# NingZhang1/pyscf_isdf

Measured on AMD Instinct MI355X. Metric: isdf_build_plus_get_jk_wall_time, lower is better.
Workload: dtype f64

## Files before the change

### include/mi355_isdf.h

```cpp
#ifndef MI355_ISDF_H
#define MI355_ISDF_H

#include <stdint.h>

#ifdef __cplusplus
extern "C" {
#endif

typedef struct isdf_ctx* isdf_handle;

#define ISDF_OK 0
#define ISDF_ERR_ARG 1
#define ISDF_ERR_HIP 2
#define ISDF_ERR_LIB 3
#define ISDF_ERR_NUM 4

int isdf_abi_version(void);

int isdf_create(int device_id, isdf_handle* out);
int isdf_destroy(isdf_handle h);
int isdf_set_stream(isdf_handle h, void* hip_stream);
const char* isdf_last_error(isdf_handle h);
int64_t isdf_workspace_bytes(isdf_handle h);
int isdf_release_workspace(isdf_handle h);
// ... 244 lines not shown
int isdf_dot(isdf_handle h, const double* d_x, const double* d_y, int64_t n, double* result);

int isdf_pack_table_pm(isdf_handle h, const double* d_tab, const int32_t mesh[3], const int32_t* d_idx, int npts, double scale,
                       double* d_s, double* d_a, int64_t ldx);
int isdf_herm_kscale_nt(isdf_handle h, int M, int N, int64_t K, double alpha, const double* d_A, int64_t lda, const double* d_B,
                        int64_t ldb, const double* d_s, const double* d_a, double beta, double* d_Cre, double* d_Cim, int64_t ldc);

int isdf_thc_pair(isdf_handle h, int P, const double* d_Xo, int64_t ldo, int no, const double* d_so, const double* d_Xv, int64_t ldv,
                  int nv, const double* d_sv, double* d_A, int64_t lda);
int isdf_trace_sq(isdf_handle h, int n, const double* d_B, int64_t ldb, double* result);

int isdf_gemm_nt(isdf_handle h, int M, int N, int64_t K, double alpha, const double* d_A, int64_t lda,
                 const double* d_B, int64_t ldb, const double* d_kscale, double beta, double* d_C,
                 int64_t ldc);

int isdf_gemm_nt_had3(isdf_handle h, int M, int N, int64_t K, double alpha, const double* d_A, int64_t lda, const double* d_H,
                      int64_t ldh, const double* d_B, int64_t ldb, int64_t bstride, double beta, double* d_C, int64_t ldc,
                      int64_t cstride);

int isdf_gemm_nn_had(isdf_handle h, int M, int64_t N, int K, double alpha, const double* d_A, int64_t lda, const double* d_H,
                     int64_t ldh, const double* d_B, int64_t ldb, double beta, double* d_C, int64_t ldc);

#ifdef __cplusplus
}
#endif
#endif
```

### pyscf_isdf_amd/backend.py

```python
import ctypes
import os
import numpy as np
import torch
from . import lib as _lib

_vp = ctypes.c_void_p


def _np_ptr(a):
    return a.ctypes.data_as(_vp)


class HipBackend:
    name = 'hip-gfx950'

    def __init__(self, device=0):
        if not torch.cuda.is_available():
            raise _lib.IsdfError('no GPU visible to torch; the ISDF path has no CPU fallback')
        self.device = torch.device('cuda', device)
        torch.cuda.set_device(self.device)
        self.handle = _lib.Handle(device)
        if os.environ.get('ISDF_TRSM') == 'subst':
            self.set_option('trsm_substitution', 1)
        if os.environ.get('ISDF_OWN_FFT') in ('0', '1', '2'):
# ... 464 lines not shown
                         B.stride(0), float(beta), self._p(C), C.stride(0))

    def hadamard_rows(self, X, Y):
        self._stream()
        self.handle.call('isdf_hadamard_rows', self._p(X), X.stride(0), self._p(Y), Y.stride(0), X.shape[0], X.shape[1])

    def gemm_nt(self, A, B, C, alpha=1.0, beta=0.0, kscale=None):
        self._stream()
        M, K = A.shape
        N = B.shape[0]
        assert B.shape[1] == K and tuple(C.shape) == (M, N) and A.stride(1) == 1 and B.stride(1) == 1 and C.stride(1) == 1
        ks = self._p(kscale) if kscale is not None else _vp(0)
        self.handle.call('isdf_gemm_nt', M, N, K, float(alpha), self._p(A), A.stride(0), self._p(B), B.stride(0), ks,
                         float(beta), self._p(C), C.stride(0))

    def gemm_nt_had3(self, A, H, B3, C3, alpha=1.0, beta=0.0):
        self._stream()
        M, K = A.shape
        N = B3.shape[1]
        assert tuple(B3.shape) == (3, N, K) and tuple(C3.shape) == (3, M, N) and A.stride(1) == 1 and B3.stride(2) == 1 and C3.stride(2) == 1
        assert H is None or (tuple(H.shape) == (M, K) and H.stride(1) == 1)
        self.handle.call('isdf_gemm_nt_had3', M, N, K, float(alpha), self._p(A), A.stride(0), self._p(H) if H is not None else _vp(0),
                         H.stride(0) if H is not None else 0, self._p(B3), B3.stride(1), B3.stride(0), float(beta), self._p(C3),
                         C3.stride(1), C3.stride(0))

    def gemm_nn_had(self, A, H, B, C, alpha=1.0, beta=0.0):
        self._stream()
        M, K = A.shape
        N = B.shape[1]
        assert tuple(B.shape) == (K, N) and tuple(H.shape) == (K, N) and tuple(C.shape) == (M, N)
# ... 310 lines not shown
```

### pyscf_isdf_amd/csrc/common.h

```cpp
#pragma once
#include <hip/hip_runtime.h>
#include <rocblas/rocblas.h>
#include <rocsolver/rocsolver.h>
#include <hipfft/hipfft.h>
#include <cstdint>
#include <cstdio>
#include <cstring>
#include <string>
#include <vector>
#include <map>
#include "../../include/mi355_isdf.h"

struct FftPlan {
  hipfftHandle fwd = 0, bwd = 0;
  size_t work_bytes = 0;
};

struct ProfRec {
  hipEvent_t e0 = nullptr, e1 = nullptr;
};
struct ProfEntry {
  std::vector<ProfRec> recs;
  double work = 0.0;
  double ms = 0.0;
// ... 9 lines not shown
};

struct isdf_ctx {
  int profiling = 0;
  std::map<std::string, ProfEntry> prof;
  int device = 0;
  hipStream_t stream = nullptr;
  rocblas_handle blas = nullptr;
  std::string err;
  std::map<std::vector<int>, FftPlan> plans;
  std::map<std::string, std::pair<void*, size_t>> ws;
  int num_cu = 256;
  int trsm_substitution = 0;
  int own_fft = 2;
  int gemm_nn_own = 0;
  int attr_gemm_b = 0, attr_gemm_nn = 0, attr_gemm_nn_had = 0, attr_gram_tri = 0, attr_herm = 0, attr_thc_pair = 0;
  int cand_gram = 1;
  int conv_pipe = 1;
  int conv_sub_rows = 0;
  int gram_pivot_tpb = 256;
  int gram_compact = 1;
  int gram_compact_permille = 875;
  int block_apply_waves = 16;
  int block_apply_reg = 1;
  double coul_omega = 0.0;
  double coul_rc = 0.0;
  int coul_sphere = 0;
  WsKernel wsk;
};

int isdf_fail(isdf_handle h, int code, const char* fmt, ...);
// ... 56 lines not shown
    if (hipEventCreate(&rec.e0) != hipSuccess || hipEventCreate(&rec.e1) != hipSuccess) { ent = nullptr; return; }
    (void)hipEventRecord(rec.e0, h->stream);
  }
  ~ProfScope() {
    if (!ent) return;
    (void)hipEventRecord(rec.e1, h->stream);
    ent->recs.push_back(rec);
  }
};

int gemm_nt_f64(isdf_handle h, int M, int N, int64_t K, double alpha, const double* A, int64_t lda,
                const double* B, int64_t ldb, double beta, double* C, int64_t ldc);
int gemm_nt_f64_scaled(isdf_handle h, int M, int N, int64_t K, double alpha, const double* A, int64_t lda,
                       const double* B, int64_t ldb, const double* kscale, double beta, double* C,
                       int64_t ldc);
int trsm_lower_left(isdf_handle h, bool trans, int m, int64_t n, const double* L, int64_t ldl, double* X, int64_t ldx);
int trsm_lower_right(isdf_handle h, bool trans, int m, int64_t n, const double* L, int64_t ldl, double* X, int64_t ldx);
int block_forward_solve(isdf_handle h, const double* D, int64_t ldd, int nblk, const int32_t* blk_off_host, double* X,
                        int64_t ldx, int64_t n, bool own_columns = false);
int block_apply_inverse(isdf_handle h, const double* Dinv, int64_t ldd, int nblk, const int32_t* blk_off_host, double* X,
                        int64_t ldx, int64_t n, bool square_input = false);
int transpose_rm(isdf_handle h, const double* src, int64_t lds, int64_t rows, int64_t cols, double* dst, int64_t ldd);
int tri_left(isdf_handle h, bool trans, int m, int64_t n, const double* L, int64_t ldl, double* X, int64_t ldx);
int tri_right(isdf_handle h, bool trans, int m, int64_t n, const double* L, int64_t ldl, double* X, int64_t ldx);
bool gemm_nn_f64_supported(isdf_handle h, int64_t M, int64_t N, int64_t K, const double* A, int64_t lda, const double* B,
                           int64_t ldb);
int gemm_nn_f64(isdf_handle h, int64_t M, int64_t N, int64_t K, const double* A, int64_t lda, const double* B, int64_t ldb,
                double* C, int64_t ldc, bool square);
int gemm_rm(isdf_handle h, char opA, char opB, int64_t M, int64_t N, int64_t K, double alpha,
            const double* A, int64_t lda, const double* B, int64_t ldb, double beta, double* C,
// ... 11 lines not shown
```

### pyscf_isdf_amd/csrc/gemm_f64.hip

```cpp
#include "common.h"
#include "gemm_tile.h"
#include <cstdlib>

int gemm_rm(isdf_handle h, char opA, char opB, int64_t M, int64_t N, int64_t K, double alpha,
            const double* A, int64_t lda, const double* B, int64_t ldb, double beta, double* C,
            int64_t ldc) {
  ARG_CHECK(h, M < 2147483647LL && N < 2147483647LL && K < 2147483647LL && lda < 2147483647LL &&
                   ldb < 2147483647LL && ldc < 2147483647LL);
  const rocblas_operation ta = (opA == 'N') ? rocblas_operation_none : rocblas_operation_transpose;
  const rocblas_operation tb = (opB == 'N') ? rocblas_operation_none : rocblas_operation_transpose;
  ProfScope ps(h, "rocblas_dgemm[flop]", 2.0 * M * N * (double)K);
  BLAS_TRY(h, rocblas_dgemm(h->blas, tb, ta, (rocblas_int)N, (rocblas_int)M, (rocblas_int)K, &alpha, B,
                            (rocblas_int)ldb, A, (rocblas_int)lda, &beta, C, (rocblas_int)ldc));
  return ISDF_OK;
}

namespace {

constexpr int BM = 128, BN = 128, BK = 16;
constexpr int LDT = 17;
constexpr int TPB = 256;

struct GemmArgs {
  const double* A; int64_t lda;
  const double* B; int64_t ldb;
  const double* kscale;
  double* P;
  int64_t ldp, slab_stride;
  int M, N;
  int64_t K, kslab;
  int ntm, ntn, nslab;
  int64_t nunits, nunits_pad;
  double alpha, beta;
  int direct;
};

#define ISDF_SLAB_STORE                                                                       \
  {                                                                                           \
    double* q = out + (int64_t)row * g.ldp + col;                                             \
    const double v = acc[i][j][r];                                                            \
    if (g.direct) *q = (g.beta == 0.0) ? g.alpha * v : g.alpha * v + g.beta * (*q);           \
    else *q = v;                                                                              \
  }

#define ISDF_MFMA16(AF, BF)                                                                   \
    _Pragma("unroll") for (int i = 0; i < 4; ++i)                                             \
      _Pragma("unroll") for (int j = 0; j < 4; ++j)                                           \
        acc[i][j] = __builtin_amdgcn_mfma_f64_16x16x4f64(AF[i], BF[j], acc[i][j], 0, 0, 0);
#define ISDF_ISSUE(XMASK, NX) _Pragma("unroll") for (int q_ = 0; q_ < 8; ++q_) {              \
    __builtin_amdgcn_sched_group_barrier(0x008, 2, 0); __builtin_amdgcn_sched_group_barrier(0x100, 1, 0);                \
    if (q_ < (NX)) __builtin_amdgcn_sched_group_barrier(XMASK, 1, 0); }

template <bool FAST>
__global__ __launch_bounds__(TPB, 2) void gemm_nt_mfma_kernel(GemmArgs g) {
  __shared__ double sA[2][BM * LDT];
  __shared__ double sB[2][BN * LDT];

  const int64_t unit = xcd_unit(g.nunits_pad);
  if (unit >= g.nunits) return;
  const Tile t = decode_tile(unit, g.ntm, g.ntn);
  const KRange kr = slab_range(t.slab, g.kslab, g.K);
  const int64_t k0 = kr.k0, k1 = kr.k1;
  const int nchunks = (int)((k1 - k0 + BK - 1) / BK);

  const int tid = threadIdx.x;
  const int lane = tid & 63, wave = tid >> 6;
  const int wm = wave >> 1, wn = wave & 1;

  const int srow = tid >> 3;
  const int sseg = tid & 7;
  const int arow0 = t.tm * BM + srow, brow0 = t.tn * BN + srow;
  const int mlast = g.M - 1, nlast = g.N - 1;
  const double* __restrict__ Ag = g.A;
  const double* __restrict__ Bg = g.B;
  const int64_t lda = g.lda, ldb = g.ldb;
// ... 59 lines not shown
    ISDF_FRAGS(3, a1, b1)
    ISDF_MFMA16(a0, b0)
    ISDF_MFMA16(a1, b1)
    if (c + 1 < nchunks) ISDF_STORE_CHUNK(buf ^ 1)
    __syncthreads();
  }
  double* out = g.P + (int64_t)t.slab * g.slab_stride;
  ISDF_STORE_ACC(4, 4, t.tm * BM + wm * 64, t.tn * BN + wn * 64, g.M, g.N, ISDF_SLAB_STORE)
#undef ISDF_LOAD_ONE
#undef ISDF_LOAD_CHUNK
#undef ISDF_STORE_ONE
#undef ISDF_STORE_CHUNK
#undef ISDF_FRAGS
}

constexpr int BM2 = 256;
constexpr int TPB2 = 512;

template <bool SCALED>
__device__ __forceinline__ void tile_256x128(const double* A, int64_t lda, const double* B, int64_t ldb, const double* kscale,
                                             int M, int N, int tm, int tn, int64_t k0, int nchunks, double* smem, d4 (&acc)[4][4]) {
  double* sA = smem;
  double* sB = smem + 2 * BM2 * LDT;
  const int last = nchunks - 1;

  const int tid = threadIdx.x;
  const int lane = tid & 63, wave = tid >> 6;
  const int wm = wave >> 1, wn = wave & 1;
  const int srow = tid >> 3;
  const int sseg = tid & 7;
// ... 81 lines not shown
    ISDF_CHUNKB(1, ISDF_LOADB(min(c + 3, last), ya0, ya1, ya2, ya3, yb0, yb1), ISDF_STOREB(0, xa0, xa1, xa2, xa3, xb0, xb1))
  }
#undef ISDF_LOADB
#undef ISDF_ST1
#undef ISDF_STOREB
#undef ISDF_FRAGQ
#undef ISDF_CHUNKB
}

template <bool SCALED>
__global__ __launch_bounds__(TPB2, 2) void gemm_nt_mfma_kernel_b(GemmArgs g) {
  extern __shared__ double smem[];
  const int64_t unit = xcd_unit(g.nunits_pad);
  if (unit >= g.nunits) return;
  const Tile t = decode_tile(unit, g.ntm, g.ntn);
  const KRange kr = slab_range(t.slab, g.kslab, g.K);
  d4 acc[4][4];
  tile_256x128<SCALED>(g.A, g.lda, g.B, g.ldb, g.kscale, g.M, g.N, t.tm, t.tn, kr.k0, (int)((kr.k1 - kr.k0) / BK), smem, acc);
  const int lane = threadIdx.x & 63, wave = threadIdx.x >> 6;
  double* out = g.P + (int64_t)t.slab * g.slab_stride;
  ISDF_STORE_ACC(4, 4, t.tm * BM2 + (wave >> 1) * 64, t.tn * BN + (wave & 1) * 64, g.M, g.N, ISDF_SLAB_STORE)
}

struct GramTriArgs {
  const double* X; int64_t ldx; int K;
  const GramTriUnit* units;
  const int64_t* blk_off;
  int64_t row0;
  const int64_t* tri_off;
  double* S;
// ... 6 lines not shown
  if (unit >= t.nunits) return;
  const GramTriUnit u = t.units[unit];
  const int64_t r0 = t.blk_off[u.blk];
  const double* X = t.X + (r0 - t.row0) * t.ldx;
  const int m = (int)(t.blk_off[u.blk + 1] - r0);
  const int64_t ldp = (int64_t)(u.tm + 1) * BM2;
  double* S = t.S + t.tri_off[u.blk] + (gram_tri_row((int64_t)u.tm * BM2) - (int64_t)u.tm * BM2 * ldp);
  d4 acc[4][4];
  tile_256x128<false>(X, t.ldx, X, t.ldx, nullptr, m, m, u.tm, u.tn, 0, t.K / BK, smem, acc);
  const int lane = threadIdx.x & 63, wave = threadIdx.x >> 6;
  ISDF_STORE_ACC(4, 4, u.tm * BM2 + (wave >> 1) * 64, u.tn * BN + (wave & 1) * 64, m, m, S[(int64_t)row * ldp + col] = acc[i][j][r];)
}

constexpr int TPBD = 256;

template <bool SCALED>
__global__ __launch_bounds__(TPBD, 2) void gemm_nt_mfma_kernel_d(GemmArgs g) {
  __shared__ double sB[2][BN * LDT];
  const int64_t unit = xcd_unit(g.nunits_pad);
  if (unit >= g.nunits) return;
  const Tile t = decode_tile(unit, g.ntm, g.ntn);
  const int tm = t.tm, tn = t.tn;
  const KRange kr = slab_range(t.slab, g.kslab, g.K);
  const int64_t k0 = kr.k0;
  const int nchunks = (int)((kr.k1 - k0) / BK);
  const int last = nchunks - 1;

  const int tid = threadIdx.x;
  const int lane = tid & 63, wave = tid >> 6;
  const int frow = lane & 15, fkq = lane >> 4;
  const int mlast = g.M - 1, nlast = g.N - 1;
  const double* pA0 = g.A + (int64_t)min(tm * BM + wave * 32 + frow, mlast) * g.lda + k0 + 4 * fkq;
  const double* pA1 = g.A + (int64_t)min(tm * BM + wave * 32 + 16 + frow, mlast) * g.lda + k0 + 4 * fkq;
  const int srow = tid >> 2, sseg = tid & 3;
  const double* pB0 = g.B + (int64_t)min(tn * BN + srow, nlast) * g.ldb + k0 + 4 * sseg;
  const double* pB1 = g.B + (int64_t)min(tn * BN + srow + 64, nlast) * g.ldb + k0 + 4 * sseg;
// ... 75 lines not shown
  __builtin_amdgcn_sched_barrier(0);
  for (int c = 0; c < nchunks; c += 2) {
    ISDF_CHUNKD(0, xa00, xa01, xa10, xa11, ISDF_LOADD(min(c + 2, last), xa00, xa01, xa10, xa11, xb00, xb01, xb10, xb11),
                ISDF_STORED(1, yb00, yb01, yb10, yb11))
    ISDF_CHUNKD(1, ya00, ya01, ya10, ya11, ISDF_LOADD(min(c + 3, last), ya00, ya01, ya10, ya11, yb00, yb01, yb10, yb11),
                ISDF_STORED(0, xb00, xb01, xb10, xb11))
  }
  double* out = g.P + (int64_t)t.slab * g.slab_stride;
  ISDF_STORE_ACC(2, 8, tm * BM + wave * 32, tn * BN, g.M, g.N, ISDF_SLAB_STORE)
#undef ISDF_LOADD
#undef ISDF_STORED
#undef ISDF_FRAGD
#undef ISDF_MFMAD
#undef ISDF_CHUNKD
}

constexpr int BN3 = 32;

struct Had3Args {
  const double* A; int64_t lda;
  const double* H; int64_t ldh;
  const double* B; int64_t ldb, bstride;
  double* P;
  int64_t ldp, pstride, slab_stride;
  int M, N;
  int64_t K, kslab;
  int ntm, ntn, nslab;
  int64_t nunits, nunits_pad;
  double alpha, beta;
  int direct;
// ... 306 lines not shown
#undef ISDF_MFMA16
#undef ISDF_ISSUE

__global__ void reduce_slabs_kernel(const double* __restrict__ P, int nslab, int64_t slab_stride,
                                    int M, int N, double alpha, double beta, double* __restrict__ C,
                                    int64_t ldc) {
  const int64_t idx = (int64_t)blockIdx.x * blockDim.x + threadIdx.x;
  if (idx >= (int64_t)M * N) return;
  const int m = (int)(idx / N), n = (int)(idx % N);
  double s = 0.0;
  for (int t = 0; t < nslab; ++t) s += P[(int64_t)t * slab_stride + idx];
  double* q = C + (int64_t)m * ldc + n;
  *q = (beta == 0.0) ? alpha * s : alpha * s + beta * (*q);
}

constexpr int TPBH = 512;

struct HermArgs {
  const double* A; int64_t lda;
  const double* B; int64_t ldb;
  const double* s; const double* a;
  double* Pre; double* Pim;
  int64_t ldp, slab_stride;
  int M, N;
  int64_t K, kslab;
  int ntm, ntn, nslab;
  int64_t nunits, nunits_pad;
  double alpha, beta;
  int direct;
};
// ... 177 lines not shown
    hipLaunchKernelGGL(herm_kscale_nt_kernel, dim3((unsigned)g.nunits_pad), dim3(TPBH), lds, h->stream, g);
    KERNEL_CHECK(h);
  }
  if (!g.direct) {
    ProfScope ps(h, "gemm_reduce_slabs_kernel[byte]", 16.0 * (double)plane * (g.nslab + 1));
    const unsigned nb = (unsigned)cdiv(plane, 256);
    hipLaunchKernelGGL(reduce_slabs_kernel, dim3(nb), dim3(256), 0, h->stream, g.Pre, g.nslab, g.slab_stride, M, N, alpha, beta,
                       d_Cre, ldc);
    hipLaunchKernelGGL(reduce_slabs_kernel, dim3(nb), dim3(256), 0, h->stream, g.Pim, g.nslab, g.slab_stride, M, N, alpha, beta,
                       d_Cim, ldc);
    KERNEL_CHECK(h);
  }
  return ISDF_OK;
}

int gemm_nt_f64_scaled(isdf_handle h, int M, int N, int64_t K, double alpha, const double* A, int64_t lda,
                       const double* B, int64_t ldb, const double* kscale, double beta, double* C,
                       int64_t ldc) {
  ARG_CHECK(h, M > 0 && N > 0 && K > 0 && A && B && C && lda >= K && ldb >= K && ldc >= N);
  GemmArgs g;
  g.A = A; g.lda = lda; g.B = B; g.ldb = ldb; g.kscale = kscale;
  g.M = M; g.N = N; g.K = K;
  static const int variant = getenv("ISDF_GEMM_VARIANT") ? atoi(getenv("ISDF_GEMM_VARIANT")) : -1;
  static const int tune = getenv("ISDF_GEMM_SLAB_TUNE") ? atoi(getenv("ISDF_GEMM_SLAB_TUNE")) : 1;
  const bool aligned = rows_aligned16(A, lda) && rows_aligned16(B, ldb) && rows_aligned16(kscale);
  const bool alignedB = aligned && K % 32 == 0, fast = aligned && K % BK == 0;
  const bool fitsB = (double)(cdiv(M, BM2) * BM2) <= 1.15 * (double)M;
  const bool useB = alignedB && M > BM && (variant == 1 || (variant == -1 && fitsB));
  const bool useD = alignedB && !useB && (variant == 3 || variant == -1);
  g.ntm = (int)cdiv(M, useB ? BM2 : BM); g.ntn = (int)cdiv(N, BN);
  const SlabPlan p = plan_slabs((int64_t)g.ntm * g.ntn, (int64_t)h->num_cu * (useB ? 1 : 2), M, N, K, 8, 2 * BK, tune != 0);
  g.kslab = p.kslab; g.nslab = p.nslab; g.nunits = p.nunits; g.nunits_pad = p.nunits_pad;
  g.alpha = alpha; g.beta = beta;
  if (g.nslab == 1) {
    g.direct = 1; g.P = C; g.ldp = ldc; g.slab_stride = 0;
  } else {
    g.direct = 0;
    g.P = (double*)isdf_ws(h, "gemm_partials", sizeof(double) * (size_t)g.nslab * M * N);
    if (!g.P) return ISDF_ERR_HIP;
    g.ldp = N; g.slab_stride = (int64_t)M * N;
  }
  ARG_CHECK(h, g.nunits_pad < 2147483647LL);
  const char* label = useD ? (kscale ? "gemm_nt_mfma_kernel_d<true>[flop]" : "gemm_nt_mfma_kernel_d<false>[flop]") : useB ? (kscale ? "gemm_nt_mfma_kernel_b<true>[flop]" : "gemm_nt_mfma_kernel_b<false>[flop]")
                           : (fast ? "gemm_nt_mfma_kernel<true>[flop]" : "gemm_nt_mfma_kernel<false>[flop]");
  {
    ProfScope ps(h, label, 2.0 * M * N * (double)K);
    if (useD) {
      if (kscale) hipLaunchKernelGGL(gemm_nt_mfma_kernel_d<true>, dim3((unsigned)g.nunits_pad), dim3(TPBD), 0, h->stream, g);
      else hipLaunchKernelGGL(gemm_nt_mfma_kernel_d<false>, dim3((unsigned)g.nunits_pad), dim3(TPBD), 0, h->stream, g);
    } else if (useB) {
      const size_t lds = sizeof(double) * 2 * (BM2 + BN) * LDT;
      if (int rc = raise_lds_once(h, h->attr_gemm_b, lds, gemm_nt_mfma_kernel_b<true>, gemm_nt_mfma_kernel_b<false>)) return rc;
      if (kscale) hipLaunchKernelGGL(gemm_nt_mfma_kernel_b<true>, dim3((unsigned)g.nunits_pad), dim3(TPB2), lds, h->stream, g);
      else hipLaunchKernelGGL(gemm_nt_mfma_kernel_b<false>, dim3((unsigned)g.nunits_pad), dim3(TPB2), lds, h->stream, g);
    } else if (fast) hipLaunchKernelGGL(gemm_nt_mfma_kernel<true>, dim3((unsigned)g.nunits_pad), dim3(TPB), 0, h->stream, g);
    else hipLaunchKernelGGL(gemm_nt_mfma_kernel<false>, dim3((unsigned)g.nunits_pad), dim3(TPB), 0, h->stream, g);
    KERNEL_CHECK(h);
  }
  if (!g.direct) {
    ProfScope ps(h, "gemm_reduce_slabs_kernel[byte]", 8.0 * (double)M * N * (g.nslab + 1));
    hipLaunchKernelGGL(reduce_slabs_kernel, dim3((unsigned)cdiv((int64_t)M * N, 256)), dim3(256), 0, h->stream,
                       g.P, g.nslab, g.slab_stride, M, N, alpha, beta, C, ldc);
    KERNEL_CHECK(h);
  }
  return ISDF_OK;
}

int gemm_nt_f64(isdf_handle h, int M, int N, int64_t K, double alpha, const double* A, int64_t lda,
                const double* B, int64_t ldb, double beta, double* C, int64_t ldc) {
  return gemm_nt_f64_scaled(h, M, N, K, alpha, A, lda, B, ldb, nullptr, beta, C, ldc);
}

extern "C" int isdf_gemm_nt(isdf_handle h, int M, int N, int64_t K, double alpha, const double* d_A,
                            int64_t lda, const double* d_B, int64_t ldb, const double* d_kscale,
                            double beta, double* d_C, int64_t ldc) {
  if (!h) return ISDF_ERR_ARG;
  return gemm_nt_f64_scaled(h, M, N, K, alpha, d_A, lda, d_B, ldb, d_kscale, beta, d_C, ldc);
}

extern "C" int isdf_gemm_nt_had3(isdf_handle h, int M, int N, int64_t K, double alpha, const double* d_A, int64_t lda,
                                 const double* d_H, int64_t ldh, const double* d_B, int64_t ldb, int64_t bstride, double beta,
                                 double* d_C, int64_t ldc, int64_t cstride) {
  if (!h) return ISDF_ERR_ARG;
  ARG_CHECK(h, M > 0 && N > 0 && K > 0 && d_A && d_B && d_C && lda >= K && (!d_H || ldh >= K) && ldb >= K && ldc >= N);
  ARG_CHECK(h, bstride >= 0 && cstride >= (int64_t)(M - 1) * ldc + N);
  const bool fused = K % BK == 0 && rows_aligned16(d_A, lda) && (!d_H || rows_aligned16(d_H, ldh)) && rows_aligned16(d_B, ldb) &&
                     bstride % 2 == 0;
  if (!fused) {
    const double* A = d_A;
    int64_t la = lda;
    if (d_H) {
      double* AH = (double*)isdf_ws(h, "had3_AH", sizeof(double) * (size_t)M * (size_t)K);
// ... 131 lines not shown
```

### pyscf_isdf_amd/csrc/gemm_tile.h

```cpp
#pragma once
#include "common.h"

namespace {

typedef double d4 __attribute__((ext_vector_type(4)));

__device__ __forceinline__ int64_t xcd_unit(int64_t nunits_pad) {
  const int64_t bid = blockIdx.x;
  const int64_t per_xcd = nunits_pad / 8;
  return (bid % 8) * per_xcd + bid / 8;
}

struct Tile { int tm, tn, slab; };
struct KRange { int64_t k0, k1; };

__device__ __forceinline__ Tile decode_tile(int64_t unit, int ntm, int ntn) {
  return {(int)(unit % ntm), (int)((unit / ntm) % ntn), (int)(unit / ((int64_t)ntm * ntn))};
}

__device__ __forceinline__ KRange slab_range(int slab, int64_t kslab, int64_t K) {
  const int64_t k0 = (int64_t)slab * kslab;
  return {k0, (k0 + kslab < K) ? k0 + kslab : K};
}

}

#define ISDF_STORE_ACC(NI, NJ, ROW0, COL0, M, N, STORE)                                       \
  _Pragma("unroll") for (int i = 0; i < NI; ++i) {                                            \
    _Pragma("unroll") for (int r = 0; r < 4; ++r) {                                           \
      const int row = ROW0 + i * 16 + (lane >> 4) + 4 * r;                                    \
      if (row >= M) continue;                                                                 \
      _Pragma("unroll") for (int j = 0; j < NJ; ++j) {                                        \
// ... 7 lines not shown
```

### pyscf_isdf_amd/csrc/jk.hip

```cpp
#include "common.h"

namespace {

constexpr int64_t JCHUNK = 32768;

__global__ void rho_reduce_kernel(const double* __restrict__ T, int64_t ldT,
                                  const double* __restrict__ ao, int64_t ld, int nao, int64_t ng,
                                  double* __restrict__ rho) {
  const int64_t g = (int64_t)blockIdx.x * blockDim.x + threadIdx.x;
  if (g >= ng) return;
  double s = 0.0;
#pragma unroll 4
  for (int mu = 0; mu < nao; ++mu) s = fma(T[(int64_t)mu * ldT + g], ao[(int64_t)mu * ld + g], s);
  rho[g] = s;
}

__global__ void hadamard_kernel(double* __restrict__ M, int64_t ldm, const double* __restrict__ W,
                                int64_t ldw, int64_t rows, int64_t cols) {
  const int64_t c = (int64_t)blockIdx.x * blockDim.x + threadIdx.x;
  const int64_t r = blockIdx.y;
  if (c >= cols) return;
  M[r * ldm + c] *= W[r * ldw + c];
}

__global__ void pair_rows_kernel(const double* __restrict__ ao, int64_t ld, const double* __restrict__ mo, int64_t ldmo,
                                 int nocc, int64_t ng, double* __restrict__ R) {
  const int64_t g = (int64_t)blockIdx.x * blockDim.x + threadIdx.x;
  if (g >= ng) return;
  const int row = blockIdx.y;
  const int i = row / nocc, jj = row % nocc;
  R[(int64_t)row * ng + g] = ao[(int64_t)i * ld + g] * mo[(int64_t)jj * ldmo + g];
// ... 4 lines not shown
  const int64_t g = (int64_t)blockIdx.x * blockDim.x + threadIdx.x;
  if (g >= ng) return;
  const int i = blockIdx.y;
  double s = 0.0;
  for (int jj = 0; jj < nocc; ++jj) s = fma(R[((int64_t)i * nocc + jj) * ng + g], mo[(int64_t)jj * ldmo + g], s);
  vdm[(int64_t)i * ng + g] = s;
}

}

extern "C" int isdf_rho(isdf_handle h, const double* d_ao, int nao, int64_t ng, int64_t ld,
                        const double* d_dm, int nset, double* d_rho, int64_t ldrho) {
  if (!h) return ISDF_ERR_ARG;
  ARG_CHECK(h, d_ao && d_dm && d_rho && nao > 0 && ng > 0 && ld >= ng && nset > 0 && ldrho >= ng);
  double* T = (double*)isdf_ws(h, "jk_T", sizeof(double) * (size_t)nao * JCHUNK);
  if (!T) return ISDF_ERR_HIP;
  for (int i = 0; i < nset; ++i) {
    for (int64_t g0 = 0; g0 < ng; g0 += JCHUNK) {
      const int64_t nc = std::min(JCHUNK, ng - g0);
      int rc = gemm_rm(h, 'N', 'N', nao, nc, nao, 1.0, d_dm + (int64_t)i * nao * nao, nao, d_ao + g0, ld, 0.0, T, JCHUNK);
      if (rc) return rc;
      hipLaunchKernelGGL(rho_reduce_kernel, dim3((unsigned)cdiv(nc, 256)), dim3(256), 0, h->stream, T, JCHUNK,
                         d_ao + g0, ld, nao, nc, d_rho + (int64_t)i * ldrho + g0);
      KERNEL_CHECK(h);
    }
  }
  return ISDF_OK;
}

extern "C" int isdf_vj_from_vR(isdf_handle h, const double* d_ao, int nao, int64_t ng, int64_t ld,
                               const double* d_vR, int nset, int64_t ldv, double* d_vj) {
  if (!h) return ISDF_ERR_ARG;
  ARG_CHECK(h, d_ao && d_vR && d_vj && nao > 0 && ng > 0 && ld >= ng && nset > 0 && ldv >= ng);
  for (int i = 0; i < nset; ++i) {
    int rc = gemm_nt_f64_scaled(h, nao, nao, ng, 1.0, d_ao, ld, d_ao, ld, d_vR + (int64_t)i * ldv, 0.0,
                                d_vj + (int64_t)i * nao * nao, nao);
    if (rc) return rc;
  }
  return ISDF_OK;
}

extern "C" int isdf_get_j(isdf_handle h, const double* d_ao, int nao, int64_t ngrids, int64_t ld,
                          const int32_t mesh[3], const double a[9], const double* d_dm, int nset,
                          double* d_vj) {
  if (!h) return ISDF_ERR_ARG;
  ARG_CHECK(h, mesh && ngrids == (int64_t)mesh[0] * mesh[1] * mesh[2]);
  double* rho = (double*)isdf_ws(h, "jk_rho", sizeof(double) * (size_t)nset * ngrids);
  if (!rho) return ISDF_ERR_HIP;
  int rc = isdf_rho(h, d_ao, nao, ngrids, ld, d_dm, nset, rho, ngrids);
  if (rc) return rc;
  rc = isdf_coulomb_potential(h, rho, nset, ngrids, mesh, a);
// ... 241 lines not shown
```

### pyscf_isdf_amd/fit_route.py

```python
import warnings
import numpy as np

_PROBE_FAILED = {
    'blockjacobi': '; rebuilding W with the Cholesky route',
    'blockjacobi-spectral': ' in the spectral build; rebuilding W the classic way',
    'blockjacobi-paneled': ' in a paneled build, where the Cholesky route is not available: rebuilding with pairs of clusters '
                           'merged into one preconditioner block'}


def spectral_line_plan(idx, scale, mesh, tile):
    idx = np.asarray(idx, dtype=np.int64)
    n0, n1, n2 = (int(x) for x in mesh)
    per = n1 * (n2 // 2 + 1)
    line, kx = idx % per, idx // per
    real = np.unique(line)
    lines = np.full(-(-len(real) // 16) * 16, -1, dtype=np.int32)
    lines[:len(real)] = real
    slot = np.full((len(lines), n0), -1, dtype=np.int32)
    where = np.searchsorted(real, line)
    slot[where, kx] = np.arange(len(idx), dtype=np.int32)
    if np.count_nonzero(slot >= 0) != len(idx):
        return None
    slot = np.ascontiguousarray(slot.reshape(-1, tile, n0).transpose(0, 2, 1))
    slot_scale = np.where(slot >= 0, np.asarray(scale, dtype=np.float64)[np.maximum(slot, 0)], 0.0)
# ... 411 lines not shown
            for j in range(n):
                be.gemm_nn(aoP, d_R[j], tmp)
                be.hadamard_rows(tmp, psiP)
                be.gemm_nn(tmp, ones, col)
                T[j].copy_(col[:, 0])
            return T
        cached = getattr(self, '_probe_R', None)
        if cached is None or cached[0] != (n, nao):
            rng = np.random.default_rng(20240203)
            R = rng.standard_normal((n, nao, nao))
            self._probe_R = ((n, nao), be.to_device(R + R.transpose(0, 2, 1)))
        d_R = self._probe_R[1]
        T = be.zeros((n, P))
        tmp = be.empty((n, P))
        for pl in planes:
            be.rho(pl, P, d_R, tmp)
            T += tmp
        return T

    def _bj_probe_vectors(self, aoT_P, Afac, Dblk, ip_off):
        T = self._bj_probe_densities(aoT_P)
        T0 = T.clone()
        self.backend.bj_probe_vectors(T, Afac, Dblk, ip_off)
        return T0, T

    def _bj_probe_energies(self, T0, F, W, grid_slice):
        be, comm = self.backend, self.comm
        cell = self.cell
        n = T0.shape[0]
        mesh = np.asarray(self.mesh, dtype=np.int32)
        G = int(np.prod(mesh))
# ... 62 lines not shown
```

### pyscf_isdf_amd/lib.py

```python
import ctypes
import os

_HERE = os.path.dirname(os.path.abspath(__file__))
LIB_PATH = os.path.join(_HERE, 'lib', 'libmi355_isdf.so')
ABI_VERSION = 21

_lib = None

c_int, c_i64, c_dbl, c_vp = ctypes.c_int, ctypes.c_int64, ctypes.c_double, ctypes.c_void_p

SIGNATURES = {
    'isdf_abi_version': (c_int, []),
    'isdf_create': (c_int, [c_int, ctypes.POINTER(c_vp)]),
    'isdf_destroy': (c_int, [c_vp]),
    'isdf_set_stream': (c_int, [c_vp, c_vp]),
    'isdf_last_error': (ctypes.c_char_p, [c_vp]),
    'isdf_workspace_bytes': (c_i64, [c_vp]),
    'isdf_set_coulomb_omega': (c_int, [c_vp, c_dbl]),
    'isdf_set_coulomb_cutoff': (c_int, [c_vp, c_dbl]),
    'isdf_set_coulomb_ws': (c_int, [c_vp, c_dbl, c_vp, c_vp, c_vp, c_vp]),
    'isdf_set_option': (c_int, [c_vp, ctypes.c_char_p, c_int]),
    'isdf_release_workspace': (c_int, [c_vp]),
    'isdf_prof_enable': (c_int, [c_vp, c_int]),
    'isdf_prof_reset': (c_int, [c_vp]),
# ... 83 lines not shown
    'isdf_mg_embed_density': (c_int, [c_vp, c_vp, c_int, c_vp, c_dbl, c_vp, c_vp, c_int]),
    'isdf_mg_restrict_potential': (c_int, [c_vp, c_vp, c_int, c_vp, c_vp, c_dbl, c_vp]),
    'isdf_mg_coulomb_kernel': (c_int, [c_vp, c_vp, c_int, c_vp, c_vp]),
    'isdf_lda_exchange': (c_int, [c_vp, c_vp, c_i64, c_vp, c_vp]),
    'isdf_lda_vwn_add': (c_int, [c_vp, c_vp, c_i64, c_vp, c_vp]),
    'isdf_gga_b88': (c_int, [c_vp, c_vp, c_vp, c_i64, c_i64, c_vp, c_vp, c_vp, c_i64]),
    'isdf_xc_fused': (c_int, [c_vp, c_vp, c_vp, c_i64, c_i64, c_dbl, c_dbl, c_dbl, c_int, c_dbl, c_vp, c_vp, c_vp, c_i64]),
    'isdf_xc_fused_rsh': (c_int, [c_vp, c_vp, c_vp, c_i64, c_i64, c_dbl, c_dbl, c_dbl, c_int, c_dbl, c_dbl, c_dbl, c_vp, c_vp, c_vp, c_i64]),
    'isdf_gga_lyp_polarised': (c_int, [c_vp, c_vp, c_vp, c_i64, c_i64, c_i64, c_dbl, c_int, c_vp, c_vp, c_vp, c_i64, c_i64]),
    'isdf_lda_exchange_fxc': (c_int, [c_vp, c_vp, c_i64, c_vp]),
    'isdf_lda_vwn_fxc_add': (c_int, [c_vp, c_vp, c_i64, c_vp]),
    'isdf_gga_b88_fxc': (c_int, [c_vp, c_vp, c_i64, c_i64, c_vp, c_i64, c_i64, c_int, c_vp, c_i64, c_i64, c_vp, c_i64]),
    'isdf_xc_fxc_apply': (c_int, [c_vp, c_int, c_vp, c_i64, c_i64, c_i64, c_vp, c_i64, c_i64, c_int, c_vp, c_i64, c_i64, c_int]),
    'isdf_dot': (c_int, [c_vp, c_vp, c_vp, c_i64, c_vp]),
    'isdf_gemm_nt': (c_int, [c_vp, c_int, c_int, c_i64, c_dbl, c_vp, c_i64, c_vp, c_i64, c_vp, c_dbl, c_vp, c_i64]),
    'isdf_gemm_nt_had3': (c_int, [c_vp, c_int, c_int, c_i64, c_dbl, c_vp, c_i64, c_vp, c_i64, c_vp, c_i64, c_i64, c_dbl, c_vp, c_i64,
                                  c_i64]),
    'isdf_gemm_nn_had': (c_int, [c_vp, c_int, c_i64, c_int, c_dbl, c_vp, c_i64, c_vp, c_i64, c_vp, c_i64, c_dbl, c_vp, c_i64]),
    'isdf_pack_table_pm': (c_int, [c_vp, c_vp, c_vp, c_vp, c_int, c_dbl, c_vp, c_vp, c_i64]),
    'isdf_herm_kscale_nt': (c_int, [c_vp, c_int, c_int, c_i64, c_dbl, c_vp, c_i64, c_vp, c_i64, c_vp, c_vp, c_dbl, c_vp, c_vp, c_i64]),
    'isdf_thc_pair': (c_int, [c_vp, c_int, c_vp, c_i64, c_int, c_vp, c_vp, c_i64, c_int, c_vp, c_vp, c_i64]),
    'isdf_trace_sq': (c_int, [c_vp, c_int, c_vp, c_i64, c_vp]),
    'isdf_get_k_exact': (c_int, [c_vp, c_vp, c_int, c_i64, c_i64, c_vp, c_int, c_vp, c_vp, c_int, c_int, c_int, c_vp]),
    'isdf_get_k': (c_int, [c_vp, c_vp, c_int, c_int, c_vp, c_i64, c_int, c_int, c_vp, c_int, c_vp]),
}


def load():
    global _lib
    if _lib is not None:
# ... 53 lines not shown
```

Baseline: 16.50.

## Exploit symmetry: upper-triangle SYRK for J potential and triangular density build

Adds a SYRK-style variant of the NT MFMA GEMM kernels. It decodes only upper-triangle tiles, reduces k-slabs only for the upper part, and then symmetrises, and it is now used for the J matrix contraction ao·diag(vR)·aoᵀ. The density build folds the symmetric density matrix into an upper-triangular form (dm + dmᵀ off the diagonal) and runs paneled GEMMs over the trapezoidal part only, cutting the flops of both steps roughly in half. The costs are extra panel GEMM launches, a symmetrisation pass, a serial loop in the tile decode, and an nao² workspace. A fit_route call is also switched to rho_pair so it does not pick up the new triangular rho path.

```diff
diff --git a/include/mi355_isdf.h b/include/mi355_isdf.h
--- a/include/mi355_isdf.h
+++ b/include/mi355_isdf.h
@@ -282,6 +282,9 @@
                  const double* d_B, int64_t ldb, const double* d_kscale, double beta, double* d_C,
                  int64_t ldc);
 
+int isdf_syrk_nt(isdf_handle h, int N, int64_t K, double alpha, const double* d_A, int64_t lda, const double* d_kscale,
+                 double* d_C, int64_t ldc, int variant);
+
 int isdf_gemm_nt_had3(isdf_handle h, int M, int N, int64_t K, double alpha, const double* d_A, int64_t lda, const double* d_H,
                       int64_t ldh, const double* d_B, int64_t ldb, int64_t bstride, double beta, double* d_C, int64_t ldc,
                       int64_t cstride);
diff --git a/pyscf_isdf_amd/backend.py b/pyscf_isdf_amd/backend.py
--- a/pyscf_isdf_amd/backend.py
+++ b/pyscf_isdf_amd/backend.py
@@ -502,6 +502,13 @@
         self.handle.call('isdf_gemm_nt', M, N, K, float(alpha), self._p(A), A.stride(0), self._p(B), B.stride(0), ks,
                          float(beta), self._p(C), C.stride(0))
 
+    def syrk_nt(self, A, C, alpha=1.0, kscale=None, variant=-1):
+        self._stream()
+        N, K = A.shape
+        assert tuple(C.shape) == (N, N) and A.stride(1) == 1 and C.stride(1) == 1
+        ks = self._p(kscale) if kscale is not None else _vp(0)
+        self.handle.call('isdf_syrk_nt', N, K, float(alpha), self._p(A), A.stride(0), ks, self._p(C), C.stride(0), int(variant))
+
     def gemm_nt_had3(self, A, H, B3, C3, alpha=1.0, beta=0.0):
         self._stream()
         M, K = A.shape
diff --git a/pyscf_isdf_amd/csrc/common.h b/pyscf_isdf_amd/csrc/common.h
--- a/pyscf_isdf_amd/csrc/common.h
+++ b/pyscf_isdf_amd/csrc/common.h
@@ -47,7 +47,7 @@
   int trsm_substitution = 0;
   int own_fft = 2;
   int gemm_nn_own = 0;
-  int attr_gemm_b = 0, attr_gemm_nn = 0, attr_gemm_nn_had = 0, attr_gram_tri = 0, attr_herm = 0, attr_thc_pair = 0;
+  int attr_gemm_b = 0, attr_gemm_nn = 0, attr_gemm_nn_had = 0, attr_gram_tri = 0, attr_herm = 0, attr_thc_pair = 0, attr_syrk_b = 0;
   int cand_gram = 1;
   int conv_pipe = 1;
   int conv_sub_rows = 0;
@@ -134,6 +134,8 @@
 int gemm_nt_f64_scaled(isdf_handle h, int M, int N, int64_t K, double alpha, const double* A, int64_t lda,
                        const double* B, int64_t ldb, const double* kscale, double beta, double* C,
                        int64_t ldc);
+int syrk_nt_f64_scaled(isdf_handle h, int N, int64_t K, double alpha, const double* A, int64_t lda, const double* kscale,
+                       double* C, int64_t ldc, int variant = -1);
 int trsm_lower_left(isdf_handle h, bool trans, int m, int64_t n, const double* L, int64_t ldl, double* X, int64_t ldx);
 int trsm_lower_right(isdf_handle h, bool trans, int m, int64_t n, const double* L, int64_t ldl, double* X, int64_t ldx);
 int block_forward_solve(isdf_handle h, const double* D, int64_t ldd, int nblk, const int32_t* blk_off_host, double* X,
diff --git a/pyscf_isdf_amd/csrc/gemm_f64.hip b/pyscf_isdf_amd/csrc/gemm_f64.hip
--- a/pyscf_isdf_amd/csrc/gemm_f64.hip
+++ b/pyscf_isdf_amd/csrc/gemm_f64.hip
@@ -33,6 +33,7 @@
   int64_t nunits, nunits_pad;
   double alpha, beta;
   int direct;
+  int ntiles;
 };
 
 #define ISDF_SLAB_STORE                                                                       \
@@ -51,14 +52,20 @@
     __builtin_amdgcn_sched_group_barrier(0x008, 2, 0); __builtin_amdgcn_sched_group_barrier(0x100, 1, 0);                \
     if (q_ < (NX)) __builtin_amdgcn_sched_group_barrier(XMASK, 1, 0); }
 
-template <bool FAST>
-__global__ __launch_bounds__(TPB, 2) void gemm_nt_mfma_kernel(GemmArgs g) {
+template <bool UPPER, int BMROWS>
+__device__ __forceinline__ Tile nt_tile(int64_t unit, const GemmArgs& g) {
+  if constexpr (UPPER) return decode_tile_upper(unit, g.ntm, g.ntiles, BMROWS, BN);
+  else return decode_tile(unit, g.ntm, g.ntn);
+}
+
+template <bool FAST, bool UPPER>
+__device__ __forceinline__ void nt_unit_a(const GemmArgs g) {
   __shared__ double sA[2][BM * LDT];
   __shared__ double sB[2][BN * LDT];
 
   const int64_t unit = xcd_unit(g.nunits_pad);
   if (unit >= g.nunits) return;
-  const Tile t = decode_tile(unit, g.ntm, g.ntn);
+  const Tile t = nt_tile<UPPER, BM>(unit, g);
   const KRange kr = slab_range(t.slab, g.kslab, g.K);
   const int64_t k0 = kr.k0, k1 = kr.k1;
   const int nchunks = (int)((k1 - k0 + BK - 1) / BK);
@@ -148,6 +155,11 @@
 #undef ISDF_FRAGS
 }
 
+template <bool FAST>
+__global__ __launch_bounds__(TPB, 2) void gemm_nt_mfma_kernel(GemmArgs g) { nt_unit_a<FAST, false>(g); }
+template <bool FAST>
+__global__ __launch_bounds__(TPB, 2) void syrk_nt_mfma_kernel(GemmArgs g) { nt_unit_a<FAST, true>(g); }
+
 constexpr int BM2 = 256;
 constexpr int TPB2 = 512;
 
@@ -259,6 +271,20 @@
   const int64_t unit = xcd_unit(g.nunits_pad);
   if (unit >= g.nunits) return;
   const Tile t = decode_tile(unit, g.ntm, g.ntn);
+  const KRange kr = slab_range(t.slab, g.kslab, g.K);
+  d4 acc[4][4];
+  tile_256x128<SCALED>(g.A, g.lda, g.B, g.ldb, g.kscale, g.M, g.N, t.tm, t.tn, kr.k0, (int)((kr.k1 - kr.k0) / BK), smem, acc);
+  const int lane = threadIdx.x & 63, wave = threadIdx.x >> 6;
+  double* out = g.P + (int64_t)t.slab * g.slab_stride;
+  ISDF_STORE_ACC(4, 4, t.tm * BM2 + (wave >> 1) * 64, t.tn * BN + (wave & 1) * 64, g.M, g.N, ISDF_SLAB_STORE)
+}
+
+template <bool SCALED>
+__global__ __launch_bounds__(TPB2, 2) void syrk_nt_mfma_kernel_b(GemmArgs g) {
+  extern __shared__ double smem[];
+  const int64_t unit = xcd_unit(g.nunits_pad);
+  if (unit >= g.nunits) return;
+  const Tile t = nt_tile<true, BM2>(unit, g);
   const KRange kr = slab_range(t.slab, g.kslab, g.K);
   d4 acc[4][4];
   tile_256x128<SCALED>(g.A, g.lda, g.B, g.ldb, g.kscale, g.M, g.N, t.tm, t.tn, kr.k0, (int)((kr.k1 - kr.k0) / BK), smem, acc);
@@ -295,12 +321,12 @@
 
 constexpr int TPBD = 256;
 
-template <bool SCALED>
-__global__ __launch_bounds__(TPBD, 2) void gemm_nt_mfma_kernel_d(GemmArgs g) {
+template <bool SCALED, bool UPPER>
+__device__ __forceinline__ void nt_unit_d(const GemmArgs g) {
   __shared__ double sB[2][BN * LDT];
   const int64_t unit = xcd_unit(g.nunits_pad);
   if (unit >= g.nunits) return;
-  const Tile t = decode_tile(unit, g.ntm, g.ntn);
+  const Tile t = nt_tile<UPPER, BM>(unit, g);
   const int tm = t.tm, tn = t.tn;
   const KRange kr = slab_range(t.slab, g.kslab, g.K);
   const int64_t k0 = kr.k0;
@@ -406,6 +432,11 @@
 #undef ISDF_MFMAD
 #undef ISDF_CHUNKD
 }
+
+template <bool SCALED>
+__global__ __launch_bounds__(TPBD, 2) void gemm_nt_mfma_kernel_d(GemmArgs g) { nt_unit_d<SCALED, false>(g); }
+template <bool SCALED>
+__global__ __launch_bounds__(TPBD, 2) void syrk_nt_mfma_kernel_d(GemmArgs g) { nt_unit_d<SCALED, true>(g); }
 
 constexpr int BN3 = 32;
 
@@ -742,6 +773,17 @@
   *q = (beta == 0.0) ? alpha * s : alpha * s + beta * (*q);
 }
 
+__global__ void reduce_slabs_upper_kernel(const double* __restrict__ P, int nslab, int64_t slab_stride, int N, double alpha,
+                                          double* __restrict__ C, int64_t ldc) {
+  const int64_t idx = (int64_t)blockIdx.x * blockDim.x + threadIdx.x;
+  if (idx >= (int64_t)N * N) return;
+  const int m = (int)(idx / N), n = (int)(idx % N);
+  if (n < m) return;
+  double s = 0.0;
+  for (int t = 0; t < nslab; ++t) s += P[(int64_t)t * slab_stride + idx];
+  C[(int64_t)m * ldc + n] = alpha * s;
+}
+
 constexpr int TPBH = 512;
 
 struct HermArgs {
@@ -949,14 +991,23 @@
   return ISDF_OK;
 }
 
-int gemm_nt_f64_scaled(isdf_handle h, int M, int N, int64_t K, double alpha, const double* A, int64_t lda,
-                       const double* B, int64_t ldb, const double* kscale, double beta, double* C,
-                       int64_t ldc) {
+namespace {
+
+int64_t upper_tile_count(int ntm, int ntn, int bm) {
+  int64_t n = 0;
+  for (int tn = 0; tn < ntn; ++tn) n += upper_tiles_in_col(tn, ntm, bm, BN);
+  return n;
+}
+
+int nt_product(isdf_handle h, int M, int N, int64_t K, double alpha, const double* A, int64_t lda, const double* B, int64_t ldb,
+               const double* kscale, double beta, double* C, int64_t ldc, bool upper, int force) {
   ARG_CHECK(h, M > 0 && N > 0 && K > 0 && A && B && C && lda >= K && ldb >= K && ldc >= N);
+  ARG_CHECK(h, !upper || (A == B && lda == ldb && M == N && beta == 0.0));
   GemmArgs g;
   g.A = A; g.lda = lda; g.B = B; g.ldb = ldb; g.kscale = kscale;
   g.M = M; g.N = N; g.K = K;
-  static const int variant = getenv("ISDF_GEMM_VARIANT") ? atoi(getenv("ISDF_GEMM_VARIANT")) : -1;
+  static const int variant_env = getenv("ISDF_GEMM_VARIANT") ? atoi(getenv("ISDF_GEMM_VARIANT")) : -1;
+  const int variant = force >= 0 ? force : variant_env;
   static const int tune = getenv("ISDF_GEMM_SLAB_TUNE") ? atoi(getenv("ISDF_GEMM_SLAB_TUNE")) : 1;
   const bool aligned = rows_aligned16(A, lda) && rows_aligned16(B, ldb) && rows_aligned16(kscale);
   const bool alignedB = aligned && K % 32 == 0, fast = aligned && K % BK == 0;
@@ -964,7 +1015,8 @@
   const bool useB = alignedB && M > BM && (variant == 1 || (variant == -1 && fitsB));
   const bool useD = alignedB && !useB && (variant == 3 || variant == -1);
   g.ntm = (int)cdiv(M, useB ? BM2 : BM); g.ntn = (int)cdiv(N, BN);
-  const SlabPlan p = plan_slabs((int64_t)g.ntm * g.ntn, (int64_t)h->num_cu * (useB ? 1 : 2), M, N, K, 8, 2 * BK, tune != 0);
+  g.ntiles = (int)(upper ? upper_tile_count(g.ntm, g.ntn, useB ? BM2 : BM) : (int64_t)g.ntm * g.ntn);
+  const SlabPlan p = plan_slabs(g.ntiles, (int64_t)h->num_cu * (useB ? 1 : 2), M, N, K, 8, 2 * BK, tune != 0);
   g.kslab = p.kslab; g.nslab = p.nslab; g.nunits = p.nunits; g.nunits_pad = p.nunits_pad;
   g.alpha = alpha; g.beta = beta;
   if (g.nslab == 1) {
@@ -978,27 +1030,62 @@
   ARG_CHECK(h, g.nunits_pad < 2147483647LL);
   const char* label = useD ? (kscale ? "gemm_nt_mfma_kernel_d<true>[flop]" : "gemm_nt_mfma_kernel_d<false>[flop]") : useB ? (kscale ? "gemm_nt_mfma_kernel_b<true>[flop]" : "gemm_nt_mfma_kernel_b<false>[flop]")
                            : (fast ? "gemm_nt_mfma_kernel<true>[flop]" : "gemm_nt_mfma_kernel<false>[flop]");
-  {
+  const char* ulabel = useD ? (kscale ? "syrk_nt_mfma_kernel_d<true>[flop]" : "syrk_nt_mfma_kernel_d<false>[flop]") : useB ? (kscale ? "syrk_nt_mfma_kernel_b<true>[flop]" : "syrk_nt_mfma_kernel_b<false>[flop]")
+                            : (fast ? "syrk_nt_mfma_kernel<true>[flop]" : "syrk_nt_mfma_kernel<false>[flop]");
+  const dim3 grid((unsigned)g.nunits_pad);
+  if (upper) {
+    ProfScope ps(h, ulabel, 2.0 * g.ntiles * (useB ? BM2 : BM) * BN * (double)K);
+    if (useD) {
+      if (kscale) hipLaunchKernelGGL(syrk_nt_mfma_kernel_d<true>, grid, dim3(TPBD), 0, h->stream, g);
+      else hipLaunchKernelGGL(syrk_nt_mfma_kernel_d<false>, grid, dim3(TPBD), 0, h->stream, g);
+    } else if (useB) {
+      const size_t lds = sizeof(double) * 2 * (BM2 + BN) * LDT;
+      if (int rc = raise_lds_once(h, h->attr_syrk_b, lds, syrk_nt_mfma_kernel_b<true>, syrk_nt_mfma_kernel_b<false>)) return rc;
+      if (kscale) hipLaunchKernelGGL(syrk_nt_mfma_kernel_b<true>, grid, dim3(TPB2), lds, h->stream, g);
+      else hipLaunchKernelGGL(syrk_nt_mfma_kernel_b<false>, grid, dim3(TPB2), lds, h->stream, g);
+    } else if (fast) hipLaunchKernelGGL(syrk_nt_mfma_kernel<true>, grid, dim3(TPB), 0, h->stream, g);
+    else hipLaunchKernelGGL(syrk_nt_mfma_kernel<false>, grid, dim3(TPB), 0, h->stream, g);
+    KERNEL_CHECK(h);
+  } else {
     ProfScope ps(h, label, 2.0 * M * N * (double)K);
     if (useD) {
-      if (kscale) hipLaunchKernelGGL(gemm_nt_mfma_kernel_d<true>, dim3((unsigned)g.nunits_pad), dim3(TPBD), 0, h->stream, g);
-      else hipLaunchKernelGGL(gemm_nt_mfma_kernel_d<false>, dim3((unsigned)g.nunits_pad), dim3(TPBD), 0, h->stream, g);
+      if (kscale) hipLaunchKernelGGL(gemm_nt_mfma_kernel_d<true>, grid, dim3(TPBD), 0, h->stream, g);
+      else hipLaunchKernelGGL(gemm_nt_mfma_kernel_d<false>, grid, dim3(TPBD), 0, h->stream, g);
     } else if (useB) {
       const size_t lds = sizeof(double) * 2 * (BM2 + BN) * LDT;
       if (int rc = raise_lds_once(h, h->attr_gemm_b, lds, gemm_nt_mfma_kernel_b<true>, gemm_nt_mfma_kernel_b<false>)) return rc;
-      if (kscale) hipLaunchKernelGGL(gemm_nt_mfma_kernel_b<true>, dim3((unsigned)g.nunits_pad), dim3(TPB2), lds, h->stream, g);
-      else hipLaunchKernelGGL(gemm_nt_mfma_kernel_b<false>, dim3((unsigned)g.nunits_pad), dim3(TPB2), lds, h->stream, g);
-    } else if (fast) hipLaunchKernelGGL(gemm_nt_mfma_kernel<true>, dim3((unsigned)g.nunits_pad), dim3(TPB), 0, h->stream, g);
-    else hipLaunchKernelGGL(gemm_nt_mfma_kernel<false>, dim3((unsigned)g.nunits_pad), dim3(TPB), 0, h->stream, g);
+      if (kscale) hipLaunchKernelGGL(gemm_nt_mfma_kernel_b<true>, grid, dim3(TPB2), lds, h->stream, g);
+      else hipLaunchKernelGGL(gemm_nt_mfma_kernel_b<false>, grid, dim3(TPB2), lds, h->stream, g);
+    } else if (fast) hipLaunchKernelGGL(gemm_nt_mfma_kernel<true>, grid, dim3(TPB), 0, h->stream, g);
+    else hipLaunchKernelGGL(gemm_nt_mfma_kernel<false>, grid, dim3(TPB), 0, h->stream, g);
     KERNEL_CHECK(h);
   }
   if (!g.direct) {
-    ProfScope ps(h, "gemm_reduce_slabs_kernel[byte]", 8.0 * (double)M * N * (g.nslab + 1));
-    hipLaunchKernelGGL(reduce_slabs_kernel, dim3((unsigned)cdiv((int64_t)M * N, 256)), dim3(256), 0, h->stream,
-                       g.P, g.nslab, g.slab_stride, M, N, alpha, beta, C, ldc);
+    if (upper) {
+      ProfScope ps(h, "gemm_reduce_slabs_upper_kernel[byte]", 4.0 * (double)M * (N + 1) * (g.nslab + 1));
+      hipLaunchKernelGGL(reduce_slabs_upper_kernel, dim3((unsigned)cdiv((int64_t)M * N, 256)), dim3(256), 0, h->stream,
+                         g.P, g.nslab, g.slab_stride, N, alpha, C, ldc);
+    } else {
+      ProfScope ps(h, "gemm_reduce_slabs_kernel[byte]", 8.0 * (double)M * N * (g.nslab + 1));
+      hipLaunchKernelGGL(reduce_slabs_kernel, dim3((unsigned)cdiv((int64_t)M * N, 256)), dim3(256), 0, h->stream,
+                         g.P, g.nslab, g.slab_stride, M, N, alpha, beta, C, ldc);
+    }
     KERNEL_CHECK(h);
   }
-  return ISDF_OK;
+  return upper ? isdf_symmetrize_upper(h, C, N, ldc) : ISDF_OK;
+}
+
+}
+
+int gemm_nt_f64_scaled(isdf_handle h, int M, int N, int64_t K, double alpha, const double* A, int64_t lda,
+                       const double* B, int64_t ldb, const double* kscale, double beta, double* C,
+                       int64_t ldc) {
+  return nt_product(h, M, N, K, alpha, A, lda, B, ldb, kscale, beta, C, ldc, false, -1);
+}
+
+int syrk_nt_f64_scaled(isdf_handle h, int N, int64_t K, double alpha, const double* A, int64_t lda, const double* kscale,
+                       double* C, int64_t ldc, int variant) {
+  return nt_product(h, N, N, K, alpha, A, lda, A, lda, kscale, 0.0, C, ldc, true, variant);
 }
 
 int gemm_nt_f64(isdf_handle h, int M, int N, int64_t K, double alpha, const double* A, int64_t lda,
@@ -1011,6 +1098,13 @@
                             double beta, double* d_C, int64_t ldc) {
   if (!h) return ISDF_ERR_ARG;
   return gemm_nt_f64_scaled(h, M, N, K, alpha, d_A, lda, d_B, ldb, d_kscale, beta, d_C, ldc);
+}
+
+extern "C" int isdf_syrk_nt(isdf_handle h, int N, int64_t K, double alpha, const double* d_A, int64_t lda,
+                            const double* d_kscale, double* d_C, int64_t ldc, int variant) {
+  if (!h) return ISDF_ERR_ARG;
+  ARG_CHECK(h, variant == -1 || variant == 0 || variant == 1 || variant == 3);
+  return syrk_nt_f64_scaled(h, N, K, alpha, d_A, lda, d_kscale, d_C, ldc, variant);
 }
 
 extern "C" int isdf_gemm_nt_had3(isdf_handle h, int M, int N, int64_t K, double alpha, const double* d_A, int64_t lda,
diff --git a/pyscf_isdf_amd/csrc/gemm_tile.h b/pyscf_isdf_amd/csrc/gemm_tile.h
--- a/pyscf_isdf_amd/csrc/gemm_tile.h
+++ b/pyscf_isdf_amd/csrc/gemm_tile.h
@@ -16,6 +16,18 @@
 
 __device__ __forceinline__ Tile decode_tile(int64_t unit, int ntm, int ntn) {
   return {(int)(unit % ntm), (int)((unit / ntm) % ntn), (int)(unit / ((int64_t)ntm * ntn))};
+}
+
+__host__ __device__ inline int upper_tiles_in_col(int tn, int ntm, int bm, int bn) {
+  const int c = ((tn + 1) * bn - 1) / bm + 1;
+  return c < ntm ? c : ntm;
+}
+
+__device__ __forceinline__ Tile decode_tile_upper(int64_t unit, int ntm, int ntiles, int bm, int bn) {
+  const int slab = (int)(unit / ntiles);
+  int idx = (int)(unit - (int64_t)slab * ntiles), tn = 0;
+  for (int c = upper_tiles_in_col(0, ntm, bm, bn); idx >= c; c = upper_tiles_in_col(++tn, ntm, bm, bn)) idx -= c;
+  return {idx, tn, slab};
 }
 
 __device__ __forceinline__ KRange slab_range(int slab, int64_t kslab, int64_t K) {
diff --git a/pyscf_isdf_amd/csrc/jk.hip b/pyscf_isdf_amd/csrc/jk.hip
--- a/pyscf_isdf_amd/csrc/jk.hip
+++ b/pyscf_isdf_amd/csrc/jk.hip
@@ -1,4 +1,5 @@
 #include "common.h"
+#include <cstdlib>
 
 namespace {
 
@@ -15,6 +16,13 @@
   rho[g] = s;
 }
 
+__global__ void rho_upper_dm_kernel(const double* __restrict__ dm, int nao, double* __restrict__ Tp) {
+  const int64_t idx = (int64_t)blockIdx.x * blockDim.x + threadIdx.x;
+  if (idx >= (int64_t)nao * nao) return;
+  const int i = (int)(idx / nao), j = (int)(idx % nao);
+  Tp[idx] = (j > i) ? dm[idx] + dm[(int64_t)j * nao + i] : (j == i) ? dm[idx] : 0.0;
+}
+
 __global__ void hadamard_kernel(double* __restrict__ M, int64_t ldm, const double* __restrict__ W,
                                 int64_t ldw, int64_t rows, int64_t cols) {
   const int64_t c = (int64_t)blockIdx.x * blockDim.x + threadIdx.x;
@@ -49,12 +57,22 @@
   if (!h) return ISDF_ERR_ARG;
   ARG_CHECK(h, d_ao && d_dm && d_rho && nao > 0 && ng > 0 && ld >= ng && nset > 0 && ldrho >= ng);
   double* T = (double*)isdf_ws(h, "jk_T", sizeof(double) * (size_t)nao * JCHUNK);
-  if (!T) return ISDF_ERR_HIP;
+  double* Tp = (double*)isdf_ws(h, "jk_Tp", sizeof(double) * (size_t)nao * nao);
+  if (!T || !Tp) return ISDF_ERR_HIP;
+  static const int panel = getenv("ISDF_RHO_PANEL") ? std::max(1, atoi(getenv("ISDF_RHO_PANEL"))) : 256;
   for (int i = 0; i < nset; ++i) {
+    hipLaunchKernelGGL(rho_upper_dm_kernel, dim3((unsigned)cdiv((int64_t)nao * nao, 256)), dim3(256), 0, h->stream,
+                       d_dm + (int64_t)i * nao * nao, nao, Tp);
+    KERNEL_CHECK(h);
     for (int64_t g0 = 0; g0 < ng; g0 += JCHUNK) {
       const int64_t nc = std::min(JCHUNK, ng - g0);
-      int rc = gemm_rm(h, 'N', 'N', nao, nc, nao, 1.0, d_dm + (int64_t)i * nao * nao, nao, d_ao + g0, ld, 0.0, T, JCHUNK);
-      if (rc) return rc;
+      for (int i0 = 0; i0 < nao; i0 += panel) {
+        const int i1 = std::min(nao, i0 + panel);
+        int rc = gemm_rm(h, 'N', 'N', i1 - i0, nc, nao - i0, 1.0, Tp + (int64_t)i0 * nao + i0, nao, d_ao + (int64_t)i0 * ld + g0, ld,
+                         0.0, T + (int64_t)i0 * JCHUNK, JCHUNK);
+        if (rc) return rc;
+      }
+      ProfScope ps(h, "rho_reduce_kernel[byte]", 8.0 * (2.0 * nao + 1.0) * (double)nc);
       hipLaunchKernelGGL(rho_reduce_kernel, dim3((unsigned)cdiv(nc, 256)), dim3(256), 0, h->stream, T, JCHUNK,
                          d_ao + g0, ld, nao, nc, d_rho + (int64_t)i * ldrho + g0);
       KERNEL_CHECK(h);
@@ -68,8 +86,7 @@
   if (!h) return ISDF_ERR_ARG;
   ARG_CHECK(h, d_ao && d_vR && d_vj && nao > 0 && ng > 0 && ld >= ng && nset > 0 && ldv >= ng);
   for (int i = 0; i < nset; ++i) {
-    int rc = gemm_nt_f64_scaled(h, nao, nao, ng, 1.0, d_ao, ld, d_ao, ld, d_vR + (int64_t)i * ldv, 0.0,
-                                d_vj + (int64_t)i * nao * nao, nao);
+    int rc = syrk_nt_f64_scaled(h, nao, ng, 1.0, d_ao, ld, d_vR + (int64_t)i * ldv, d_vj + (int64_t)i * nao * nao, nao);
     if (rc) return rc;
   }
   return ISDF_OK;
diff --git a/pyscf_isdf_amd/fit_route.py b/pyscf_isdf_amd/fit_route.py
--- a/pyscf_isdf_amd/fit_route.py
+++ b/pyscf_isdf_amd/fit_route.py
@@ -449,7 +449,7 @@
         T = be.zeros((n, P))
         tmp = be.empty((n, P))
         for pl in planes:
-            be.rho(pl, P, d_R, tmp)
+            be.rho_pair(pl, pl, P, d_R, tmp)
             T += tmp
         return T
 
diff --git a/pyscf_isdf_amd/lib.py b/pyscf_isdf_amd/lib.py
--- a/pyscf_isdf_amd/lib.py
+++ b/pyscf_isdf_amd/lib.py
@@ -121,6 +121,7 @@
     'isdf_xc_fxc_apply': (c_int, [c_vp, c_int, c_vp, c_i64, c_i64, c_i64, c_vp, c_i64, c_i64, c_int, c_vp, c_i64, c_i64, c_int]),
     'isdf_dot': (c_int, [c_vp, c_vp, c_vp, c_i64, c_vp]),
     'isdf_gemm_nt': (c_int, [c_vp, c_int, c_int, c_i64, c_dbl, c_vp, c_i64, c_vp, c_i64, c_vp, c_dbl, c_vp, c_i64]),
+    'isdf_syrk_nt': (c_int, [c_vp, c_int, c_i64, c_dbl, c_vp, c_i64, c_vp, c_vp, c_i64, c_int]),
     'isdf_gemm_nt_had3': (c_int, [c_vp, c_int, c_int, c_i64, c_dbl, c_vp, c_i64, c_vp, c_i64, c_vp, c_i64, c_i64, c_dbl, c_vp, c_i64,
                                   c_i64]),
     'isdf_gemm_nn_had': (c_int, [c_vp, c_int, c_i64, c_int, c_dbl, c_vp, c_i64, c_vp, c_i64, c_vp, c_i64, c_dbl, c_vp, c_i64]),
```

Result: no change. 16.37 (median of 6 runs) (-0.8%).
